# unknownue/puflow

Measured on AMD Instinct MI355X. Metric: patches/sec x4 2048->8192 (PU1K discrete, eval), higher is better.
Workload: dtype f32 (split-fp16 MFMA products, fp32 accumulate); 1 GPU; BASELINE configs[1]: PU1K discrete x4 inference, 32 x 2048-pt patches per GPU (fp32-parity mode); patches_per_gpu=32, total_batch=32, npoint=2048

## Files before the change

### include/puflow_hip.h

```cpp
#ifndef PUFLOW_HIP_H
#define PUFLOW_HIP_H

#ifdef __cplusplus
extern "C" {
#endif

#define PF_OK 0
#define PF_ERR_NULL (-1)
#define PF_ERR_SHAPE (-2)
#define PF_ERR_UNSUPPORTED (-3)
#define PF_ERR_LAUNCH (-4)
#define PF_ERR_WORKSPACE (-5)

int pf_version(void);
const char* pf_error_string(int code);

int pf_knn(const float* p1, const float* p2, int B, int N, int M, int K, int* idx_out, float* dist_out, void* stream);

int pf_nn1(const float* p1, const float* p2, int B, int N, int M, float* dist_out, int* idx_out, void* stream);

int pf_edgeconv(int cfg, const float* pq_or_xyz, const float* tab, const int* idx, const float* wfrag, float* out,
                int B, int N, void* stream);

int pf_edgeconv_tuned(int cfg, int variant, const float* pq_or_xyz, const float* tab, const int* idx,
                      const float* wfrag, float* out, int B, int N, void* stream);

int pf_edgeconv_pq(int unit, const float* pq_or_xyz, const int* idx, const float* wfrag, float* out, const float* w,
                   const long long* off, float* pq_next, int B, int N, int fuse, void* stream);

int pf_pq_gemm(int unit, const float* h, const float* w, const long long* off, float* pq_next, int T, void* stream);
int pf_cond(int unit, const float* h, const float* w, const long long* off, float* c, float* st, float* cp, int T,
            void* stream);
int pf_post(int unit, const float* h, const float* w, const long long* off, float* c, float* st, float* cp,
            float* pq_next, int T, void* stream);
int pf_test_act_pairn(const float* x, int n, float inv, float slope, unsigned* old_h, unsigned* old_l, unsigned* new_h,
                      unsigned* new_l, void* stream);
int pf_cond_all(const float* const* h, const float* w, const long long* off, float* const* c, float* st, float* cp, int T,
                void* stream);

int pf_flow_fwd(const float* xyz, const float* cp, const float* st, const float* w, float* z, float* ld_pt, int T,
                void* stream);

int pf_flow_inv(const float* u, const float* cp, const float* st, const float* w, float* x, int T, int R, void* stream);

int pf_logp(const float* z, const float* ld_pt, float ld_const, int B, int N, float* ldj, float* lpsum, float* logp,
            void* stream);

long long pf_flow_fwd_logp_ws_floats(int B, int N);
int pf_flow_fwd_logp(const float* xyz, const float* cp, const float* st, const float* w, float* z, float* ld_pt,
                     float ld_const, int B, int N, float* ldj, float* lpsum, float* logp, float* ws, void* stream);

int pf_interp(const float* xyz, const float* z, const int* idx16, const float* w, const long long* off, float* u_out,
              int B, int N, int R, void* stream);

int pf_interp_weights(const float* xyz, const int* idx16, const float* w, const long long* off, float* aw_out, int B, int N,
                      void* stream);
int pf_flow_inv_interp(const float* aw, const float* z, const int* idx16, const float* cp, const float* st, const float* w,
                       float* x, int B, int N, int R, void* stream);

int pf_chamfer_fwd(const float* x, const float* y, int B, int N, int M, float* dist1, int* idx1, float* dist2,
                   int* idx2, float* per_sample, float* mean_sum, void* stream);

int pf_chamfer_bwd(const float* x, const float* y, const int* idx1, const int* idx2, const float* g1, const float* g2,
                   float* gx, float* gy, int B, int N, int M, void* stream);
int pf_chamfer_bwd_det(const float* x, const float* y, const int* idx1, const int* idx2, const float* g1, const float* g2,
                       float* gx, float* gy, int B, int N, int M, void* stream);

int pf_emd_forward(const float* xyz1, const float* xyz2, float* dist, int* assignment, float* price,
                   int* assignment_inv, int* bid, float* bid_increments, float* max_increments, int* unass_idx,
                   int* max_idx, float eps, int iters, int B, int n, void* stream);

int pf_emd_forward_ex(const float* xyz1, const float* xyz2, float* dist, int* assignment, float* price,
                      int* assignment_inv, int* bid, float* bid_increments, float* max_increments, int* unass_idx,
                      int* max_idx, float eps, int iters, int B, int n, int groups, unsigned* status, void* stream);

int pf_emd_backward(const float* xyz1, const float* xyz2, float* gradxyz, const float* graddist, const int* idx, int B,
                    int n, void* stream);


long long pf_gemm_ws_floats(int M, int N, int K);
int pf_gemm(const float* A, long long sam, long long sak, const float* B, long long sbk, long long sbn, float* C,
// ... 405 lines not shown
```

### puflow_amd/csrc/flow.hip

```cpp
#include <hip/hip_runtime.h>
#include "pf_api_internal.h"
#include "pf_mfma.h"
#include "pf_wave.h"

#ifndef PF_FLOW_NW
#define PF_FLOW_NW 16
#endif
#ifndef PF_FLOW_NW_FWD
#define PF_FLOW_NW_FWD 16
#endif

namespace {

constexpr int FLOW_REC = 5360;
constexpr float LOG2PI_F = 1.8378770664093453f;

struct FlowArgs {
    const float* in;
    const float* cp;
    const float* st;
    const float* w;
    float* out;
    float* ld_pt;
    int T;
// ... 40 lines not shown
            v.z = fmaf(wb.x, h1[0], v.z); v.w = fmaf(wb.z, h1[0], v.w);
            if (TD == 2) {
                v.x = fmaf(wa.y, h1[1], v.x); v.y = fmaf(wa.w, h1[1], v.y);
                v.z = fmaf(wb.y, h1[1], v.z); v.w = fmaf(wb.w, h1[1], v.w);
            }
            hid[cb] = v;
        }
        hp[0][0] = pf_act_pairn(hid[0], hid[1], 0.01f);
        hp[0][1] = pf_act_pairn(hid[2], hid[3], 0.01f);
    }
    const PfW2Lds ws{reinterpret_cast<const u4*>(rec), lane};
    f4 h2[1][4];
#pragma unroll
    for (int ob = 0; ob < 4; ++ob) h2[0][ob] = pf_bias(rec + 5120, ob, q);
    pf_mmn<false, 4, 2, 2>(ws, 0, hp, h2);
    hp[0][0] = pf_act_pairn(h2[0][0], h2[0][1], i2, 0.01f);
    hp[0][1] = pf_act_pairn(h2[0][2], h2[0][3], i2, 0.01f);
    f4 acc[1][1];
    acc[0][0] = *reinterpret_cast<const f4*>(rec + 5184 + 4 * q);
    pf_mmn<false, 1, 2, 2>(ws, 8, hp, acc);
    o[0] = acc[0][0].x * i4; o[1] = acc[0][0].y * i4;
}

template <bool INV, int NW>
__global__ __launch_bounds__(NW * 64) void flow_kernel(FlowArgs a) {
    const int lane = threadIdx.x & 63, wave = threadIdx.x >> 6;
    const int col = lane & 15, q = lane >> 4;
    __shared__ f4 wl[6 * FLOW_REC / 4];
    pf_stage_lds(wl, reinterpret_cast<const f4*>(a.w), 6 * FLOW_REC / 4);
    __syncthreads();
    const float* wlf = reinterpret_cast<const float*>(wl);

    for (int tile = blockIdx.x; tile < a.ntiles; tile += gridDim.x) {
        const int g = (tile * NW + wave) * 16 + col;
        const bool ok = g < a.rows;
        const int row = ok ? g : a.rows - 1;
        const int pt = row / a.R;
        float v[3], ld = 0.f;
        if (INV && a.aw) {
            const int r = row - pt * a.R, bN = (pt / a.N) * a.N;
            const int4 j0 = *reinterpret_cast<const int4*>(a.idx + (size_t)pt * 16), j1 = *reinterpret_cast<const int4*>(a.idx + (size_t)pt * 16 + 4);
            const int jj[8] = {j0.x, j0.y, j0.z, j0.w, j1.x, j1.y, j1.z, j1.w};
            float sk[8][3];
#pragma unroll
            for (int k = 0; k < 8; ++k) {
                const float wk = a.aw[((size_t)pt * 8 + k) * 4 + r];
                const float* zz = a.z + (size_t)(bN + jj[k]) * 3;
// ... 10 lines not shown
        }
        FlowCond cn = flow_cond(a.cp, a.st, a.T, INV ? 5 : 0, pt, q);

        pf_static_for<0, 6>([&](auto uc) {
            constexpr int i = decltype(uc)::value;
            constexpr int u = INV ? 5 - i : i;
            constexpr int TD = (u % 2 == 0) ? 1 : 2;
            const float* rec = wlf + u * FLOW_REC;
            const float* fc = rec + 5328;
            const FlowCond c = cn;
            if constexpr (i < 5) cn = flow_cond(a.cp, a.st, a.T, INV ? u - 1 : u + 1, pt, q);
            __builtin_amdgcn_sched_barrier(0);
            const float s[3] = {c.s0.x, c.s0.y, c.s0.z}, t[3] = {c.s0.w, c.s1.x, c.s1.y};
            float h1[2], o[2];
            if constexpr (!INV) {
                const float x0 = v[0], x1 = v[1], x2 = v[2];
#pragma unroll
                for (int k = 0; k < 3; ++k)
                    v[k] = fmaf(fc[3 * k + 2], x2, fmaf(fc[3 * k + 1], x1, fmaf(fc[3 * k], x0, fc[9 + k])));
                h1[0] = v[0]; h1[1] = v[1];
                coupling_net<TD>(rec, lane, q, c, h1, o);
                if (TD == 1) { v[1] -= o[0]; v[2] -= o[1]; } else { v[2] -= o[0]; }
                const float y0 = v[2], y1 = v[1], y2 = v[0];
                v[0] = (y0 - t[0]) * expf(-s[0]);
                v[1] = (y1 - t[1]) * expf(-s[1]);
                v[2] = (y2 - t[2]) * expf(-s[2]);
                ld -= (s[0] + s[1]) + s[2];
            } else {
                const float y0 = fmaf(v[0], expf(s[0]), t[0]);
                const float y1 = fmaf(v[1], expf(s[1]), t[1]);
                const float y2 = fmaf(v[2], expf(s[2]), t[2]);
                v[0] = y2; v[1] = y1; v[2] = y0;
                h1[0] = v[0]; h1[1] = v[1];
                coupling_net<TD>(rec, lane, q, c, h1, o);
                if (TD == 1) { v[1] += o[0]; v[2] += o[1]; } else { v[2] += o[0]; }
                const float x0 = v[0], x1 = v[1], x2 = v[2];
#pragma unroll
                for (int k = 0; k < 3; ++k)
                    v[k] = fmaf(fc[12 + 3 * k + 2], x2, fmaf(fc[12 + 3 * k + 1], x1, fmaf(fc[12 + 3 * k], x0, fc[21 + k])));
            }
        });

        if (ok && q == 0) {
            a.out[(size_t)row * 3 + 0] = v[0];
            a.out[(size_t)row * 3 + 1] = v[1];
            a.out[(size_t)row * 3 + 2] = v[2];
            if (!INV) a.ld_pt[row] = ld;
        }
        if constexpr (!INV) {
            if (a.part) {
                float sl = ld;
                float sz = -0.5f * (v[0] * v[0] + LOG2PI_F) + -0.5f * (v[1] * v[1] + LOG2PI_F) + -0.5f * (v[2] * v[2] + LOG2PI_F);
                sl += __shfl_xor(sl, 1); sz += __shfl_xor(sz, 1);
                sl += __shfl_xor(sl, 2); sz += __shfl_xor(sz, 2);
// ... 23 lines not shown
            for (int i = lane; i < per; i += 64) {
                accl += PF_LD(a.part + b * per + i);
                accz += PF_LD(a.part + half + b * per + i);
            }
            accl = pf_xor_sum<32, 1>(accl); accz = pf_xor_sum<32, 1>(accz);
            if (lane == 0) {
                const float l = accl + a.ld_const * (float)a.N;
                a.ldj[b] = l;
                a.lps[b] = accz + l;
                if (b < NW * 64) sa[b] = accz + l;
            }
        }
        __syncthreads();
        float tot = 0.f;
        if (tid == 0)
            for (int b = 0; b < a.B; ++b) tot += b < NW * 64 ? sa[b] : a.lps[b];
        if (tid == 0) {
            *a.logp = -tot / (float)a.B;
            PF_ST(a.counter, 0u);
        }
    }
}

template <bool INV, int NW>
int launch_nw(FlowArgs a, hipStream_t s) {
    a.ntiles = (a.rows + NW * 16 - 1) / (NW * 16);
    const int grid = a.ntiles < 256 ? a.ntiles : 256;
    hipLaunchKernelGGL((flow_kernel<INV, NW>), dim3(grid), dim3(NW * 64), 0, s, a);
    return pf_last_launch_status();
}

template <bool INV>
int launch(FlowArgs a, hipStream_t s) {
    constexpr int NWMAX = INV ? PF_FLOW_NW : PF_FLOW_NW_FWD;
    const int wt = (a.rows + 15) / 16;
    if (wt >= 200 * NWMAX) return launch_nw<INV, NWMAX>(a, s);
    if (wt >= 200 * 8) return launch_nw<INV, 8>(a, s);
    return launch_nw<INV, 4>(a, s);
}

__global__ __launch_bounds__(256) void logp_batch_kernel(const float* __restrict__ z, const float* __restrict__ ld_pt,
                                                        float ld_const, int N, float* __restrict__ ldj,
                                                        float* __restrict__ lpsum) {
    __shared__ float sa[256], sb[256];
    const int b = blockIdx.x, tid = threadIdx.x;
    float accl = 0.f, accz = 0.f;
    for (int n = tid; n < N; n += 256) {
        accl += ld_pt[(size_t)b * N + n];
        const float* zz = z + ((size_t)b * N + n) * 3;
        accz += -0.5f * (zz[0] * zz[0] + LOG2PI_F) + -0.5f * (zz[1] * zz[1] + LOG2PI_F) + -0.5f * (zz[2] * zz[2] + LOG2PI_F);
    }
    sa[tid] = accl; sb[tid] = accz;
    __syncthreads();
    for (int s = 128; s > 0; s >>= 1) {
        if (tid < s) { sa[tid] += sa[tid + s]; sb[tid] += sb[tid + s]; }
        __syncthreads();
    }
    if (tid == 0) {
        const float l = sa[0] + ld_const * (float)N;
        ldj[b] = l;
        lpsum[b] = sb[0] + l;
    }
}

__global__ void logp_final_kernel(const float* __restrict__ lpsum, int B, float* __restrict__ logp) {
    if (threadIdx.x == 0 && blockIdx.x == 0) {
        float s = 0.f;
        for (int b = 0; b < B; ++b) s += lpsum[b];
        *logp = -s / (float)B;
    }
}

}

extern "C" int pf_flow_fwd(const float* xyz, const float* cp, const float* st, const float* w, float* z, float* ld_pt,
                           int T, void* stream) {
    if (!xyz || !cp || !st || !w || !z || !ld_pt) return PF_ERR_NULL;
    if (T <= 0) return PF_ERR_SHAPE;
    FlowArgs a{};
    a.in = xyz; a.cp = cp; a.st = st; a.w = w; a.out = z; a.ld_pt = ld_pt; a.T = T; a.R = 1; a.rows = T;
    return launch<false>(a, (hipStream_t)stream);
}

extern "C" long long pf_flow_fwd_logp_ws_floats(int B, int N) { return 2ll * (((long long)B * N + 15) / 16) + 4; }

extern "C" int pf_flow_fwd_logp(const float* xyz, const float* cp, const float* st, const float* w, float* z, float* ld_pt,
                                float ld_const, int B, int N, float* ldj, float* lpsum, float* logp, float* ws, void* stream) {
    if (!xyz || !cp || !st || !w || !z || !ld_pt || !ldj || !lpsum || !logp || !ws) return PF_ERR_NULL;
    if (B <= 0 || N <= 0 || (long long)B * N > (1ll << 30)) return PF_ERR_SHAPE;
    const int T = B * N;
    if (N % 16 != 0) {
        const int rc = pf_flow_fwd(xyz, cp, st, w, z, ld_pt, T, stream);
        return rc != PF_OK ? rc : pf_logp(z, ld_pt, ld_const, B, N, ldj, lpsum, logp, stream);
    }
    FlowArgs a{};
    a.in = xyz; a.cp = cp; a.st = st; a.w = w; a.out = z; a.ld_pt = ld_pt; a.T = T; a.R = 1; a.rows = T;
    a.part = ws; a.counter = reinterpret_cast<unsigned*>(ws + 2 * (T / 16));
    a.ldj = ldj; a.lps = lpsum; a.logp = logp; a.ld_const = ld_const; a.B = B; a.N = N;
    return launch<false>(a, (hipStream_t)stream);
}

extern "C" int pf_flow_inv(const float* u, const float* cp, const float* st, const float* w, float* x, int T, int R,
                           void* stream) {
    if (!u || !cp || !st || !w || !x) return PF_ERR_NULL;
    if (T <= 0 || R <= 0 || (long long)T * R > (1ll << 30)) return PF_ERR_SHAPE;
    FlowArgs a{};
    a.in = u; a.cp = cp; a.st = st; a.w = w; a.out = x; a.ld_pt = nullptr; a.T = T; a.R = R; a.rows = T * R;
    return launch<true>(a, (hipStream_t)stream);
}

extern "C" int pf_flow_inv_interp(const float* aw, const float* z, const int* idx16, const float* cp, const float* st, const float* w,
                                  float* x, int B, int N, int R, void* stream) {
    if (!aw || !z || !idx16 || !cp || !st || !w || !x) return PF_ERR_NULL;
    if (B <= 0 || N < 8 || (long long)B * N * R > (1ll << 30)) return PF_ERR_SHAPE;
    if (R < 1 || R > 4) return PF_ERR_UNSUPPORTED;
    FlowArgs a{};
    a.in = nullptr; a.cp = cp; a.st = st; a.w = w; a.out = x; a.ld_pt = nullptr; a.T = B * N; a.R = R; a.rows = B * N * R;
    a.aw = aw; a.z = z; a.idx = idx16; a.N = N;
    return launch<true>(a, (hipStream_t)stream);
}

extern "C" int pf_logp(const float* z, const float* ld_pt, float ld_const, int B, int N, float* ldj, float* lpsum,
                       float* logp, void* stream) {
    if (!z || !ld_pt || !ldj || !lpsum || !logp) return PF_ERR_NULL;
    if (B <= 0 || N <= 0) return PF_ERR_SHAPE;
    hipStream_t s = (hipStream_t)stream;
    hipLaunchKernelGGL(logp_batch_kernel, dim3(B), dim3(256), 0, s, z, ld_pt, ld_const, N, ldj, lpsum);
    hipLaunchKernelGGL(logp_final_kernel, dim3(1), dim3(64), 0, s, lpsum, B, logp);
    return pf_last_launch_status();
}
```

### puflow_amd/csrc/interp.hip

```cpp
#include <hip/hip_runtime.h>
#include "pf_api_internal.h"
#include "pf_mfma.h"
#include "pf_wave.h"

#ifndef PF_INTERP_P
#define PF_INTERP_P 1
#endif
#ifndef PF_INTERP_NW
#define PF_INTERP_NW 12
#endif

namespace {

struct InterpArgs {
    const float* xyz;
    const float* z;
    const int* idx;
    const float* w;
    long long off[15];
    float* u;
    float* aw;
    int T, N, ntiles, R;
    int per;
    int contiguous;
};

template <int P, int NW, bool BIG = false>
__global__ __launch_bounds__(NW * 64) void interp_kernel(InterpArgs a) {
    constexpr int R = 4;
    const int lane = threadIdx.x & 63, wave = threadIdx.x >> 6;
    const int col = lane & 15, q = lane >> 4;
    const int ps = col >> 3, k = col & 7;
    constexpr int L_DT = 0, L_ET = 2, L_WT = 6, L_D3 = 10, L_EC = 18, L_D6 = 34, L_W3 = 50, L_END = 66;
    __shared__ u4 wl[L_END * 128];
    {
        auto stage = [&](int f0, int nf, long long off) {
            const u4* src = reinterpret_cast<const u4*>(a.w + off);
            pf_stage_lds(wl + f0 * 128, src, nf * 128);
        };
        if (a.contiguous) stage(L_DT, L_END, a.off[0]);
        else {
            stage(L_DT, 2, a.off[0]); stage(L_ET, 4, a.off[5]); stage(L_WT, 4, a.off[8]); stage(L_D3, 8, a.off[1]);
            stage(L_EC, 16, a.off[6]); stage(L_D6, 16, a.off[3]); stage(L_W3, 16, a.off[9]);
        }
        __syncthreads();
    }
    const PfW1Lds wsDT{wl + L_DT * 128, lane}, wsET{wl + L_ET * 128, lane}, wsWT{wl + L_WT * 128, lane};
    const PfW2Lds wsD3{wl + L_D3 * 128, lane}, wsEC{wl + L_EC * 128, lane}, wsD6{wl + L_D6 * 128, lane}, wsW3{wl + L_W3 * 128, lane};
    const PfW2BufD<4> wsW0(a.w + a.off[7], lane);
    const PfW2BufD<2> wsW6(a.w + a.off[BIG ? 13 : 11], lane);

    const float* sc = a.w + a.off[4];
    const float iDT = sc[0], iD3 = sc[1], iW1 = sc[2], iEC = sc[3], iW3 = sc[4], iW6 = sc[5];

    const int wt_end = min((int)(blockIdx.x + 1) * a.per, a.ntiles);
    for (int wt = blockIdx.x * a.per + wave; wt < wt_end; wt += NW) {
        const int pt0 = wt * P * 2;
        int gi[P], gj[P];
        bool ok[P];
        h8 e[P];
#pragma unroll
        for (int p = 0; p < P; ++p) {
            const int g = pt0 + p * 2 + ps;
            ok[p] = g < a.T;
            gi[p] = ok[p] ? g : a.T - 1;
            gj[p] = (gi[p] / a.N) * a.N + a.idx[(size_t)gi[p] * 16 + k];
            float xi[3], xj[3];
#pragma unroll
            for (int c = 0; c < 3; ++c) {
                xi[c] = a.xyz[(size_t)gi[p] * 3 + c];
                xj[c] = a.xyz[(size_t)gj[p] * 3 + c];
            }
            const float v0 = xi[0] - xj[0], v1 = xi[1] - xj[1], v2 = xi[2] - xj[2];
            const float nrm = sqrtf(__fadd_rn(__fadd_rn(__fmul_rn(v0, v0), __fmul_rn(v1, v1)), __fmul_rn(v2, v2)));
            const f4 e0 = {xi[0], xi[1], xi[2], xj[0]}, e1 = {xj[1], xj[2], nrm, 1.f};
            e[p] = pf_edge_operand(e0, e1, q);
        }

        f4 w1[P][8];
// ... 193 lines not shown
```

### puflow_amd/csrc/pointwise.hip

```cpp
#include <hip/hip_runtime.h>
#include "pf_api_internal.h"
#include "pf_mfma.h"
#include "pf_pq.h"

namespace {

struct PqArgs {
    const float* h;
    const u4* w;
    const float* bias;
    const float* scales;
    float* pq;
    int T, ntiles, NT, nrounds;
    float inv;
};

template <int ODIM, int ROWS, int NW>
__global__ __launch_bounds__(NW * 64) void pq_gemm_kernel(PqArgs a) {
    constexpr int HB = ODIM / 16, CP = (HB + 1) / 2, OBT = ROWS / 16, RB = OBT / NW, NTMAX = 16;
    static_assert(OBT % NW == 0, "rows split evenly over the waves");
    const int lane = threadIdx.x & 63, wave = threadIdx.x >> 6;
    const int col = lane & 15, q = lane >> 4;
    __shared__ u4 bl[NTMAX * PQ_TILE_U4<CP>];
    h8 wh[RB][CP], wl[RB][CP];
// ... 25 lines not shown
        __syncthreads();
    }
}

template <int ODIM, int ROWS, int NW>
int launch_pq(PqArgs a, hipStream_t s) {
    a.ntiles = (a.T + 15) / 16;
    int nt = a.ntiles / 256;
    nt = nt < 1 ? 1 : (nt > 16 ? 16 : nt);
    a.NT = nt;
    a.nrounds = (a.ntiles + nt - 1) / nt;
    const int grid = a.nrounds < 256 ? a.nrounds : 256;
    hipLaunchKernelGGL((pq_gemm_kernel<ODIM, ROWS, NW>), dim3(grid), dim3(NW * 64), 0, s, a);
    return pf_last_launch_status();
}

struct CondArgs {
    const float* h;
    const float* w;
    long long off[13];
    float* c;
    float* st;
    float* cp;
    int T, ntiles;
    int contiguous;
};

__device__ __forceinline__ f4 pf_scale(f4 v, float k) { return v * k; }

template <int ODIM>
constexpr int cond_lds_bytes() { return ((ODIM / 32) * ((ODIM / 16 + 1) / 2) + 12 * ((ODIM / 32 + 1) / 2) + 20) * 2048; }

template <int ODIM, int CDIM, int NW>
__device__ __forceinline__ void cond_body(const CondArgs& a, u4* wl, int tile0, int tstride) {
    constexpr int HB = ODIM / 16, MB = ODIM / 32, CB = CDIM / 16;
    constexpr int HP = (HB + 1) / 2, MP = (MB + 1) / 2;
    constexpr int F_M1 = 0, F_H1 = F_M1 + MB * HP, F_S2 = F_H1 + 12 * MP, F_T2 = F_S2 + 8, F_ST4 = F_T2 + 8, F_END = F_ST4 + 4;
    const int lane = threadIdx.x & 63, wave = threadIdx.x >> 6;
    const int col = lane & 15, q = lane >> 4;
    static_assert(F_END * 2048 == cond_lds_bytes<ODIM>(), "LDS size formula");
    {
        auto stage = [&](int f0, int nf, long long off) {
            const u4* src = reinterpret_cast<const u4*>(a.w + off);
            pf_stage_lds(wl + f0 * 128, src, nf * 128);
        };
        if (a.contiguous) stage(F_M1, F_END, a.off[0]);
// ... 30 lines not shown
        }
        PfPairN mp[1][MP];
        {
            f4 m[1][MB + (MB & 1)];
#pragma unroll
            for (int o = 0; o < MB; ++o) m[0][o] = pf_bias(b1, o, q);
            pf_mmn<false, MB, HP, HP>(wsM1, 0, hp, m);
#pragma unroll
            for (int c = 0; c < MP; ++c) {
                if (2 * c + 1 < MB) mp[0][c] = pf_relu_pairn(m[0][2 * c], m[0][2 * c + 1], iM1);
                else mp[0][c] = pf_join_halfn(pf_relu_halfn(m[0][2 * c], iM1), PfHalfN{});
            }
        }
        if (a.c) {
            f4 c[1][CB];
#pragma unroll
            for (int o = 0; o < CB; ++o) c[0][o] = pf_splat(0.f);
            pf_mmn<false, CB, MP, MP>(wsM2, 0, mp, c);
            if (ok)
#pragma unroll
                for (int o = 0; o < CB; ++o)
                    *reinterpret_cast<f4*>(a.c + (size_t)pt * CDIM + o * 16 + 4 * q) = pf_scale(c[0][o], iM2);
        }
        if (!a.st) continue;
        {
            f4 acc[1][4];
#pragma unroll
            for (int o = 0; o < 4; ++o) acc[0][o] = pf_splat(0.f);
            pf_mmn<false, 4, MP, MP>(wsH1, 8 * MP, mp, acc);
            if (ok)
#pragma unroll
                for (int o = 0; o < 4; ++o)
                    *reinterpret_cast<f4*>(a.cp + (size_t)pt * 64 + o * 16 + 4 * q) = pf_scale(acc[0][o], iH1);
        }
        PfPairN h2p[1][4];
        pf_static_for<0, 2>([&](auto nc) {
            constexpr int net = decltype(nc)::value;
            f4 h1[1][4];
#pragma unroll
            for (int o = 0; o < 4; ++o) h1[0][o] = pf_splat(0.f);
            pf_mmn<false, 4, MP, MP>(wsH1, (4 * net) * MP, mp, h1);
            PfPairN h1p[1][2];
            h1p[0][0] = pf_act_pairn(h1[0][0], h1[0][1], iH1, 0.01f);
            h1p[0][1] = pf_act_pairn(h1[0][2], h1[0][3], iH1, 0.01f);
            f4 h2[1][4];
#pragma unroll
            for (int o = 0; o < 4; ++o) h2[0][o] = pf_bias(net == 0 ? bS2 : bT2, o, q);
            if constexpr (net == 0) pf_mmn<false, 4, 2, 2>(wsS2, 0, h1p, h2); else pf_mmn<false, 4, 2, 2>(wsT2, 0, h1p, h2);
            const float i2 = net == 0 ? iS2 : iT2;
            h2p[0][2 * net + 0] = pf_act_pairn(h2[0][0], h2[0][1], i2, 0.01f);
            h2p[0][2 * net + 1] = pf_act_pairn(h2[0][2], h2[0][3], i2, 0.01f);
        });
        {
            f4 acc[1][1];
            acc[0][0] = pf_bias(bST4, 0, q);
            pf_mmn<false, 1, 4, 4>(wsST4, 0, h2p, acc);
            if (ok && q < 2) *reinterpret_cast<f4*>(a.st + (size_t)pt * 8 + 4 * q) = pf_scale(acc[0][0], iST4);
        }
    }
}

#ifndef PF_COND_NW
#define PF_COND_NW 12
#endif
constexpr int COND_NW = PF_COND_NW;

template <int ODIM, int CDIM>
__global__ __launch_bounds__(COND_NW * 64) void cond_kernel(CondArgs a) {
    extern __shared__ u4 cond_lds[];
    cond_body<ODIM, CDIM, COND_NW>(a, cond_lds, blockIdx.x, gridDim.x);
}

struct CondAllArgs { CondArgs u[6]; int first[7]; };

__global__ __launch_bounds__(COND_NW * 64) void cond_all_kernel(CondAllArgs g) {
    extern __shared__ u4 cond_lds[];
    const int b = blockIdx.x;
    int unit = 0;
#pragma unroll
    for (int i = 1; i < 6; ++i) unit += b >= g.first[i] ? 1 : 0;
// ... 65 lines not shown
        case 32: return launch_pq<32, 288, 9>(a, s);
        case 64: return launch_pq<64, 288, 9>(a, s);
        case 128: return launch_pq<128, 288, 9>(a, s);
        default: return PF_ERR_UNSUPPORTED;
    }
}

extern "C" int pf_cond(int unit, const float* h, const float* w, const long long* off, float* c, float* st, float* cp,
                       int T, void* stream) {
    if (!h || !w || !off || !st || !cp) return PF_ERR_NULL;
    if (T <= 0) return PF_ERR_SHAPE;
    CondArgs a{};
    a.h = h; a.w = w; a.c = c; a.st = st; a.cp = cp; a.T = T;
    for (int i = 0; i < 13; ++i) a.off[i] = off[i];
    hipStream_t s = (hipStream_t)stream;
    switch (unit) {
        case 0: return launch_cond<32, 32>(a, s);
        case 1: return launch_cond<64, 64>(a, s);
        case 2: case 3: case 4: case 5: return launch_cond<128, 128>(a, s);
        default: return PF_ERR_UNSUPPORTED;
    }
}

extern "C" int pf_cond_all(const float* const* h, const float* w, const long long* off, float* const* c, float* st, float* cp,
                           int T, void* stream) {
    if (!h || !w || !off || (!st != !cp) || (!st && !c)) return PF_ERR_NULL;
    if (T <= 0) return PF_ERR_SHAPE;
    CondAllArgs g{};
    const int ntiles = (T + 15) / 16;
    const int wgt = (ntiles + COND_NW - 1) / COND_NW;
    static const int share_big[6] = {32, 32, 48, 48, 48, 48}, share_small[6] = {24, 32, 50, 50, 50, 50};
    const int* share = wgt <= 50 ? share_small : share_big;
    g.first[0] = 0;
    for (int u = 0; u < 6; ++u) {
        if (!h[u]) return PF_ERR_NULL;
        CondArgs& a = g.u[u];
        a.h = h[u]; a.w = w; a.c = c ? c[u] : nullptr; a.st = st ? st + (size_t)u * T * 8 : nullptr; a.cp = cp ? cp + (size_t)u * T * 64 : nullptr; a.T = T;
        a.ntiles = ntiles;
        for (int i = 0; i < 13; ++i) a.off[i] = off[u * 13 + i];
        a.contiguous = cond_contiguous(a.off, u == 0 ? 32 : (u == 1 ? 64 : 128));
        const int n = wgt < share[u] ? wgt : share[u];
        g.first[u + 1] = g.first[u] + n;
    }
    constexpr int lds = cond_lds_bytes<128>();
    allow_lds(cond_all_kernel, lds);
    hipLaunchKernelGGL(cond_all_kernel, dim3(g.first[6]), dim3(COND_NW * 64), lds, (hipStream_t)stream, g);
    return pf_last_launch_status();
}

extern "C" int pf_post(int unit, const float* h, const float* w, const long long* off, float* c, float* st, float* cp,
                       float* pq_next, int T, void* stream) {
    if (unit < 5) {
        if (!pq_next) return PF_ERR_NULL;
        const int rc = pf_pq_gemm(unit, h, w, off, pq_next, T, stream);
        if (rc != PF_OK) return rc;
    }
    return pf_cond(unit, h, w, off, c, st, cp, T, stream);
}

namespace {
__global__ void act_pairn_test_kernel(const float* __restrict__ x, int n8, float inv, float slope, u4* __restrict__ old_h,
                                      u4* __restrict__ old_l, u4* __restrict__ new_h, u4* __restrict__ new_l) {
    const int i = blockIdx.x * blockDim.x + threadIdx.x;
    if (i >= n8) return;
    const f4 b0 = *reinterpret_cast<const f4*>(x + (size_t)i * 8), b1 = *reinterpret_cast<const f4*>(x + (size_t)i * 8 + 4);
    const PfPairN o = pf_pairn(pf_lrelu(pf_scale(b0, inv), slope), pf_lrelu(pf_scale(b1, inv), slope));
    const PfPairN n = inv == 1.f ? pf_act_pairn(b0, b1, slope) : pf_act_pairn(b0, b1, inv, slope);
    old_h[i] = __builtin_bit_cast(u4, o.h); old_l[i] = __builtin_bit_cast(u4, o.l);
    new_h[i] = __builtin_bit_cast(u4, n.h); new_l[i] = __builtin_bit_cast(u4, n.l);
}
// ... 13 lines not shown
```

### puflow_amd/interpflow.py

```python
from __future__ import annotations

import os
from typing import List, Optional, Tuple

import numpy as np
import torch
import torch.nn as nn
from torch import Tensor

from . import _lib
from .packing import COND_CHANNELS, FEAT_CHANNELS, GROWTH, NUM_BLOCKS, fold_state_dict, pack_plan

_EC_CFG = [0, 1, 2, 2, 2, 2]
_CHECK_FINITE = os.environ.get("PF_CHECK_FINITE", "0") == "1"


def _conv_bn(cin: int, cout: int, slope: float) -> nn.Sequential:
    return nn.Sequential(nn.Conv2d(cin, cout, kernel_size=1), nn.BatchNorm2d(cout), nn.LeakyReLU(slope))


class _EdgeConvParams(nn.Module):

    def __init__(self, cin: int, odim: int, growth: int):
        super().__init__()
        nconv = odim // growth
        self.convs = nn.ModuleList([_conv_bn(3 * cin + growth * t, growth, 0.05) for t in range(nconv)])
# ... 50 lines not shown
        self.coupling1.bias_net = _CondNet(tdim + cdim, hdim, idim - tdim)
        self.coupling2 = _Holder()
        self.coupling2.bias_net = _CondNet(cdim, hdim, idim)
        self.coupling2.scale_net = _CondNet(cdim, hdim, idim)


class _InterpParams(nn.Module):

    def __init__(self):
        super().__init__()
        self.knn_context = _Holder()
        self.knn_context.distance_encoder = _Holder()
        self.knn_context.distance_encoder.mlp = nn.Sequential(
            *_conv_bn(10, 64, 0.01), *_conv_bn(64, 64, 0.01), nn.Conv2d(64, 128, kernel_size=1))
        self.knn_context.feat_conv = _EdgeConvParams(3, 128, 16)
        self.weight_unit = _Holder()
        self.weight_unit.mlp = nn.Sequential(
            *_conv_bn(256, 128, 0.01), *_conv_bn(128, 64, 0.01), nn.Conv2d(64, 32, kernel_size=1))


class CondList(list):
    cp: Tensor
    st: Tensor


def _host_state_dict(sd):
    out, groups = {}, {}
    for k, v in sd.items():
        v = v.detach()
        if v.is_cuda:
            groups.setdefault(v.dtype, []).append((k, v))
        else:
            out[k] = v
    for dt, items in groups.items():
        flat = torch.cat([v.reshape(-1) for _, v in items]).cpu()
        pos = 0
        for k, v in items:
            out[k] = flat[pos:pos + v.numel()].reshape(v.shape)
            pos += v.numel()
    return {k: out[k] for k in sd}


class _Engine:
    def __init__(self, sd, device: torch.device, ec_mode: Optional[str] = None):
        sd = _host_state_dict(sd)
        self.lib = _lib.load()
# ... 51 lines not shown
        for u in range(NUM_BLOCKS):
            h = torch.empty((T, FEAT_CHANNELS[u + 1]), dtype=torch.float32, device=dev)
            src = xyz.data_ptr() if u == 0 else (pq if u % 2 else pq2).data_ptr()
            nxt = pq2 if u % 2 else pq

            def ec(u=u, src=src, h=h):
                self._edgeconv(u, src, idx16, h, B, N, s)

            def ec_pq(u=u, src=src, h=h, nxt=nxt):
                w = self.ec1n_w[u] if u < 2 else self.ec4_w[u]
                _lib.check(self.lib.pf_edgeconv_pq(u, src, idx16.data_ptr(), self._p(w), h.data_ptr(), self.base, self.post[u],
                                                   nxt.data_ptr(), B, N, self.fuse_pq, s), f"pf_edgeconv_pq[{u}]")

            def pq_gemm(u=u, h=h, nxt=nxt):
                _lib.check(self.lib.pf_pq_gemm(u, h.data_ptr(), self.base, self.post[u], nxt.data_ptr(), T, s), f"pf_pq_gemm[{u}]")

            if u + 1 == NUM_BLOCKS:
                yield h, [(f"edgeconv{u}", ec)]
            elif fused:
                yield h, [(f"edgeconv{u}+pq", ec_pq)]
            else:
                yield h, [(f"edgeconv{u}", ec), (f"pq{u}", pq_gemm)]

    def features(self, xyz: Tensor, idx16: Tensor, want_cs: bool, cs_only: bool = False):
        B, N, _ = xyz.shape
        T, dev, s = B * N, xyz.device, self._stream()
        cp = torch.empty((NUM_BLOCKS, T, 64), dtype=torch.float32, device=dev) if not (cs_only and want_cs) else None
        st = torch.empty((NUM_BLOCKS, T, 8), dtype=torch.float32, device=dev) if not (cs_only and want_cs) else None
        hs: List[Tensor] = []
        for h, calls in self._unit_chain(xyz, idx16):
            for _, call in calls:
                call()
            hs.append(h)
        cs: List[Optional[Tensor]] = [torch.empty((B, N, COND_CHANNELS[u]), dtype=torch.float32, device=dev) if want_cs else None
                                      for u in range(NUM_BLOCKS)]
        self._cond_all(hs, cs if want_cs else None, st, cp, T, s)
        return (cs if want_cs else None), cp, st

    def _cond_all(self, hs, cs, st: Optional[Tensor], cp: Optional[Tensor], T: int, s) -> None:
        import ctypes
        PtrArr = ctypes.c_void_p * NUM_BLOCKS
        h_arr = PtrArr(*[h.data_ptr() for h in hs])
        c_arr = PtrArr(*[c.data_ptr() for c in cs]) if cs is not None else None
        _lib.check(self.lib.pf_cond_all(h_arr, self.base, self.post_all, c_arr, st.data_ptr() if st is not None else None,
                                        cp.data_ptr() if cp is not None else None, T, s), "pf_cond_all")

    def logp_ws(self, B: int, N: int, dev) -> Tensor:
        return torch.zeros((int(self.lib.pf_flow_fwd_logp_ws_floats(B, N)),), dtype=torch.float32, device=dev)

    def flow_f(self, xyz: Tensor, cp: Tensor, st: Tensor, ws: Optional[Tensor] = None):
        B, N, _ = xyz.shape
        T, dev, s = B * N, xyz.device, self._stream()
        z = torch.empty((B, N, 3), dtype=torch.float32, device=dev)
        ld_pt = torch.empty((T,), dtype=torch.float32, device=dev)
        ldj = torch.empty((B,), dtype=torch.float32, device=dev)
        lps = torch.empty((B,), dtype=torch.float32, device=dev)
        logp = torch.empty((), dtype=torch.float32, device=dev)
        if ws is None:
            key = (B, N, s)
            ws = self._logp_ws.get(key)
            if ws is None:
                ws = self._logp_ws[key] = self.logp_ws(B, N, dev)
        _lib.check(self.lib.pf_flow_fwd_logp(xyz.data_ptr(), cp.data_ptr(), st.data_ptr(), self._p(self.flow), z.data_ptr(),
                                             ld_pt.data_ptr(), self.ld_const, B, N, ldj.data_ptr(), lps.data_ptr(), logp.data_ptr(),
                                             ws.data_ptr(), s), "pf_flow_fwd_logp")
        return z, ldj, logp

    def interp(self, xyz: Tensor, z: Tensor, idx16: Tensor, R: int) -> Tensor:
        B, N, _ = xyz.shape
        u = torch.empty((B, N * R, 3), dtype=torch.float32, device=xyz.device)
        _lib.check(self.lib.pf_interp(xyz.data_ptr(), z.data_ptr(), idx16.data_ptr(), self.base, self.interp_off,
                                      u.data_ptr(), B, N, R, self._stream()), "pf_interp")
        return u

    def interp_weights(self, xyz: Tensor, idx16: Tensor) -> Tensor:
        B, N, _ = xyz.shape
        aw = torch.empty((B * N, 8, 4), dtype=torch.float32, device=xyz.device)
        _lib.check(self.lib.pf_interp_weights(xyz.data_ptr(), idx16.data_ptr(), self.base, self.interp_off, aw.data_ptr(), B, N,
                                              self._stream()), "pf_interp_weights")
        return aw

    def flow_g_interp(self, aw: Tensor, z: Tensor, idx16: Tensor, cp: Tensor, st: Tensor, R: int) -> Tensor:
        B, N, _ = z.shape
        x = torch.empty((B, N * R, 3), dtype=torch.float32, device=z.device)
        _lib.check(self.lib.pf_flow_inv_interp(aw.data_ptr(), z.data_ptr(), idx16.data_ptr(), cp.data_ptr(), st.data_ptr(),
                                               self._p(self.flow), x.data_ptr(), B, N, R, self._stream()), "pf_flow_inv_interp")
        return x

    def side_stream(self) -> "torch.cuda.Stream":
        if self._side is None:
            self._side = torch.cuda.Stream(device=self.device)
        return self._side

    def split_interp_for(self, T: int, R: int) -> bool:
        return R <= 4 and self.split_interp == 1

    def flow_g(self, u: Tensor, cp: Tensor, st: Tensor, R: int) -> Tensor:
        B, NR, _ = u.shape
        T = B * NR // R
        x = torch.empty_like(u)
        _lib.check(self.lib.pf_flow_inv(u.data_ptr(), cp.data_ptr(), st.data_ptr(), self._p(self.flow), x.data_ptr(),
                                        T, R, self._stream()), "pf_flow_inv")
        return x


    def profile_stages(self, xyz: Tensor, iters: int = 5, R: int = 4) -> dict:
        B, N, _ = xyz.shape
        T, dev, s = B * N, xyz.device, self._stream()
        acc: dict = {}

        def timed(name, fn):
            a, b = torch.cuda.Event(enable_timing=True), torch.cuda.Event(enable_timing=True)
            a.record()
            r = fn()
            b.record()
            acc.setdefault(name, []).append((a, b))
            return r

        for _ in range(iters + 1):
            idx16 = timed("knn", lambda: self.knn(xyz))
            cp = torch.empty((NUM_BLOCKS, T, 64), dtype=torch.float32, device=dev)
            st = torch.empty((NUM_BLOCKS, T, 8), dtype=torch.float32, device=dev)
            hs = []
            for h, calls in self._unit_chain(xyz, idx16, split_two_launch=True):
                for name, call in calls:
# ... 108 lines not shown
        u = torch.flatten(self._prep(z).transpose(2, 3), 1, 2).contiguous()
        return self._engine(upratio).flow_g(u, cs.cp, cs.st, upratio)

    def forward(self, xyz: Tensor, upratio: int = 4) -> Tuple[Tensor, Tensor]:
        if self.training:
            from .train_ops import forward_train
            if not xyz.is_cuda:
                raise _lib.PuflowHipError("input must be a GPU tensor (no CPU fallback)")
            self._train_forwards = getattr(self, "_train_forwards", 0) + 1
            return forward_train(self, xyz, upratio)
        with torch.no_grad():
            return self._forward_eval(xyz, upratio)

    def _forward_eval(self, xyz: Tensor, upratio: int, ws: Optional[Tensor] = None) -> Tuple[Tensor, Tensor]:
        self._check_mode()
        xyz = self._prep(xyz)
        e = self._engine(upratio)
        idx16 = e.knn(xyz)
        if e.split_interp_for(xyz.shape[0] * xyz.shape[1], upratio):
            main, side = torch.cuda.current_stream(), e.side_stream()
            side.wait_stream(main)
            with torch.cuda.stream(side):
                aw = e.interp_weights(xyz, idx16)
            _, cp, st = e.features(xyz, idx16, want_cs=False)
            z, _, logp = e.flow_f(xyz, cp, st, ws)
            main.wait_stream(side)
            aw.record_stream(main)
            x = e.flow_g_interp(aw, z, idx16, cp, st, upratio)
        else:
            _, cp, st = e.features(xyz, idx16, want_cs=False)
            z, _, logp = e.flow_f(xyz, cp, st, ws)
            u = e.interp(xyz, z, idx16, upratio)
            x = e.flow_g(u, cp, st, upratio)
        if _CHECK_FINITE and not bool(torch.isfinite(x).all() & torch.isfinite(logp)):
            raise _lib.PuflowHipError("non-finite output: an activation left the fp16 range of the split-fp16 kernels "
                                      "(or the input holds NaN/inf); check the input normalisation (patch.py:168-178)")
        return x, logp

    @torch.no_grad()
    def forward_stages(self, xyz: Tensor, upratio: int = 4) -> dict:
        self._check_mode()
        xyz = self._prep(xyz)
        e = self._engine(upratio)
        idx16 = e.knn(xyz)
        cs, cp, st = e.features(xyz, idx16, want_cs=True)
        z, ldj, logp = e.flow_f(xyz, cp, st)
        u = e.interp(xyz, z, idx16, upratio)
        x = e.flow_g(u, cp, st, upratio)
        B, N, _ = xyz.shape
        fz = u.view(B, N, upratio, 3).transpose(2, 3)
        return dict(idx16=idx16, cs=cs, cp=cp, st=st, z=z, ldj=ldj, logp=logp, fz=fz, x=x)

    def sample(self, sparse: Tensor, upratio: int = 4) -> Tensor:
# ... 40 lines not shown
```

Before: 28520 patches/s.

## Precompute flow scale exponentials and log-det in cond kernel; dynamic interp tile scheduling

The conditioning kernel now also writes per-point records holding exp(s) or exp(-s), the shift terms and the summed log-determinant, in separate forward and inverse layouts. The forward and inverse flow kernels read these records instead of calling expf per coupling step, and the inverse runs R times per point, so the same exponentials were being recomputed. The interp kernel also switches from a static per-wave tile stride to an LDS atomic counter for dynamic tile assignment. This adds two extra T×8 record buffers per block to write and read, and the atomic adds some contention.

```diff
diff --git a/include/puflow_hip.h b/include/puflow_hip.h
--- a/include/puflow_hip.h
+++ b/include/puflow_hip.h
@@ -37,6 +37,8 @@
                       unsigned* new_l, void* stream);
 int pf_cond_all(const float* const* h, const float* w, const long long* off, float* const* c, float* st, float* cp, int T,
                 void* stream);
+int pf_cond_all_rec(const float* const* h, const float* w, const long long* off, float* const* c, float* st, float* cp,
+                    float* rec_f, float* rec_g, int T, void* stream);
 
 int pf_flow_fwd(const float* xyz, const float* cp, const float* st, const float* w, float* z, float* ld_pt, int T,
                 void* stream);
@@ -57,6 +59,13 @@
                       void* stream);
 int pf_flow_inv_interp(const float* aw, const float* z, const int* idx16, const float* cp, const float* st, const float* w,
                        float* x, int B, int N, int R, void* stream);
+
+int pf_flow_fwd_logp_rec(const float* xyz, const float* cp, const float* rec_f, const float* w, float* z, float* ld_pt,
+                         float ld_const, int B, int N, float* ldj, float* lpsum, float* logp, float* ws, void* stream);
+int pf_flow_inv_rec(const float* u, const float* cp, const float* rec_g, const float* w, float* x, int T, int R, void* stream);
+int pf_flow_inv_interp_rec(const float* aw, const float* z, const int* idx16, const float* cp, const float* rec_g,
+                           const float* w, float* x, int B, int N, int R, void* stream);
+int pf_test_flow_expf(const float* x, int n, float* y, void* stream);
 
 int pf_chamfer_fwd(const float* x, const float* y, int B, int N, int M, float* dist1, int* idx1, float* dist2,
                    int* idx2, float* per_sample, float* mean_sum, void* stream);
diff --git a/puflow_amd/csrc/flow.hip b/puflow_amd/csrc/flow.hip
--- a/puflow_amd/csrc/flow.hip
+++ b/puflow_amd/csrc/flow.hip
@@ -86,7 +86,7 @@
     o[0] = acc[0][0].x * i4; o[1] = acc[0][0].y * i4;
 }
 
-template <bool INV, int NW>
+template <bool INV, bool REC, int NW>
 __global__ __launch_bounds__(NW * 64) void flow_kernel(FlowArgs a) {
     const int lane = threadIdx.x & 63, wave = threadIdx.x >> 6;
     const int col = lane & 15, q = lane >> 4;
@@ -143,14 +143,21 @@
                 coupling_net<TD>(rec, lane, q, c, h1, o);
                 if (TD == 1) { v[1] -= o[0]; v[2] -= o[1]; } else { v[2] -= o[0]; }
                 const float y0 = v[2], y1 = v[1], y2 = v[0];
-                v[0] = (y0 - t[0]) * expf(-s[0]);
-                v[1] = (y1 - t[1]) * expf(-s[1]);
-                v[2] = (y2 - t[2]) * expf(-s[2]);
-                ld -= (s[0] + s[1]) + s[2];
+                if constexpr (REC) {
+                    v[0] = (y0 - t[0]) * s[0];
+                    v[1] = (y1 - t[1]) * s[1];
+                    v[2] = (y2 - t[2]) * s[2];
+                    ld += c.s1.z;
+                } else {
+                    v[0] = (y0 - t[0]) * expf(-s[0]);
+                    v[1] = (y1 - t[1]) * expf(-s[1]);
+                    v[2] = (y2 - t[2]) * expf(-s[2]);
+                    ld -= (s[0] + s[1]) + s[2];
+                }
             } else {
-                const float y0 = fmaf(v[0], expf(s[0]), t[0]);
-                const float y1 = fmaf(v[1], expf(s[1]), t[1]);
-                const float y2 = fmaf(v[2], expf(s[2]), t[2]);
+                const float y0 = fmaf(v[0], REC ? s[0] : expf(s[0]), t[0]);
+                const float y1 = fmaf(v[1], REC ? s[1] : expf(s[1]), t[1]);
+                const float y2 = fmaf(v[2], REC ? s[2] : expf(s[2]), t[2]);
                 v[0] = y2; v[1] = y1; v[2] = y0;
                 h1[0] = v[0]; h1[1] = v[1];
                 coupling_net<TD>(rec, lane, q, c, h1, o);
@@ -220,21 +227,26 @@
     }
 }
 
-template <bool INV, int NW>
+template <bool INV, bool REC, int NW>
 int launch_nw(FlowArgs a, hipStream_t s) {
     a.ntiles = (a.rows + NW * 16 - 1) / (NW * 16);
     const int grid = a.ntiles < 256 ? a.ntiles : 256;
-    hipLaunchKernelGGL((flow_kernel<INV, NW>), dim3(grid), dim3(NW * 64), 0, s, a);
+    hipLaunchKernelGGL((flow_kernel<INV, REC, NW>), dim3(grid), dim3(NW * 64), 0, s, a);
     return pf_last_launch_status();
 }
 
-template <bool INV>
-int launch(FlowArgs a, hipStream_t s) {
+template <bool INV, bool REC>
+int launch_rec(FlowArgs a, hipStream_t s) {
     constexpr int NWMAX = INV ? PF_FLOW_NW : PF_FLOW_NW_FWD;
     const int wt = (a.rows + 15) / 16;
-    if (wt >= 200 * NWMAX) return launch_nw<INV, NWMAX>(a, s);
-    if (wt >= 200 * 8) return launch_nw<INV, 8>(a, s);
-    return launch_nw<INV, 4>(a, s);
+    if (wt >= 200 * NWMAX) return launch_nw<INV, REC, NWMAX>(a, s);
+    if (wt >= 200 * 8) return launch_nw<INV, REC, 8>(a, s);
+    return launch_nw<INV, REC, 4>(a, s);
+}
+
+template <bool INV>
+int launch(FlowArgs a, bool rec, hipStream_t s) {
+    return rec ? launch_rec<INV, true>(a, s) : launch_rec<INV, false>(a, s);
 }
 
 __global__ __launch_bounds__(256) void logp_batch_kernel(const float* __restrict__ z, const float* __restrict__ ld_pt,
@@ -271,51 +283,100 @@
 
 }
 
-extern "C" int pf_flow_fwd(const float* xyz, const float* cp, const float* st, const float* w, float* z, float* ld_pt,
-                           int T, void* stream) {
+static int flow_fwd(const float* xyz, const float* cp, const float* st, bool rec, const float* w, float* z, float* ld_pt,
+                    int T, void* stream) {
     if (!xyz || !cp || !st || !w || !z || !ld_pt) return PF_ERR_NULL;
     if (T <= 0) return PF_ERR_SHAPE;
     FlowArgs a{};
     a.in = xyz; a.cp = cp; a.st = st; a.w = w; a.out = z; a.ld_pt = ld_pt; a.T = T; a.R = 1; a.rows = T;
-    return launch<false>(a, (hipStream_t)stream);
+    return launch<false>(a, rec, (hipStream_t)stream);
+}
+
+extern "C" int pf_flow_fwd(const float* xyz, const float* cp, const float* st, const float* w, float* z, float* ld_pt,
+                           int T, void* stream) {
+    return flow_fwd(xyz, cp, st, false, w, z, ld_pt, T, stream);
 }
 
 extern "C" long long pf_flow_fwd_logp_ws_floats(int B, int N) { return 2ll * (((long long)B * N + 15) / 16) + 4; }
 
-extern "C" int pf_flow_fwd_logp(const float* xyz, const float* cp, const float* st, const float* w, float* z, float* ld_pt,
-                                float ld_const, int B, int N, float* ldj, float* lpsum, float* logp, float* ws, void* stream) {
+static int flow_fwd_logp(const float* xyz, const float* cp, const float* st, bool rec, const float* w, float* z, float* ld_pt,
+                         float ld_const, int B, int N, float* ldj, float* lpsum, float* logp, float* ws, void* stream) {
     if (!xyz || !cp || !st || !w || !z || !ld_pt || !ldj || !lpsum || !logp || !ws) return PF_ERR_NULL;
     if (B <= 0 || N <= 0 || (long long)B * N > (1ll << 30)) return PF_ERR_SHAPE;
     const int T = B * N;
     if (N % 16 != 0) {
-        const int rc = pf_flow_fwd(xyz, cp, st, w, z, ld_pt, T, stream);
+        const int rc = flow_fwd(xyz, cp, st, rec, w, z, ld_pt, T, stream);
         return rc != PF_OK ? rc : pf_logp(z, ld_pt, ld_const, B, N, ldj, lpsum, logp, stream);
     }
     FlowArgs a{};
     a.in = xyz; a.cp = cp; a.st = st; a.w = w; a.out = z; a.ld_pt = ld_pt; a.T = T; a.R = 1; a.rows = T;
     a.part = ws; a.counter = reinterpret_cast<unsigned*>(ws + 2 * (T / 16));
     a.ldj = ldj; a.lps = lpsum; a.logp = logp; a.ld_const = ld_const; a.B = B; a.N = N;
-    return launch<false>(a, (hipStream_t)stream);
-}
-
-extern "C" int pf_flow_inv(const float* u, const float* cp, const float* st, const float* w, float* x, int T, int R,
-                           void* stream) {
+    return launch<false>(a, rec, (hipStream_t)stream);
+}
+
+extern "C" int pf_flow_fwd_logp(const float* xyz, const float* cp, const float* st, const float* w, float* z, float* ld_pt,
+                                float ld_const, int B, int N, float* ldj, float* lpsum, float* logp, float* ws, void* stream) {
+    return flow_fwd_logp(xyz, cp, st, false, w, z, ld_pt, ld_const, B, N, ldj, lpsum, logp, ws, stream);
+}
+
+extern "C" int pf_flow_fwd_logp_rec(const float* xyz, const float* cp, const float* rec_f, const float* w, float* z, float* ld_pt,
+                                    float ld_const, int B, int N, float* ldj, float* lpsum, float* logp, float* ws, void* stream) {
+    return flow_fwd_logp(xyz, cp, rec_f, true, w, z, ld_pt, ld_const, B, N, ldj, lpsum, logp, ws, stream);
+}
+
+static int flow_inv(const float* u, const float* cp, const float* st, bool rec, const float* w, float* x, int T, int R,
+                    void* stream) {
     if (!u || !cp || !st || !w || !x) return PF_ERR_NULL;
     if (T <= 0 || R <= 0 || (long long)T * R > (1ll << 30)) return PF_ERR_SHAPE;
     FlowArgs a{};
     a.in = u; a.cp = cp; a.st = st; a.w = w; a.out = x; a.ld_pt = nullptr; a.T = T; a.R = R; a.rows = T * R;
-    return launch<true>(a, (hipStream_t)stream);
-}
-
-extern "C" int pf_flow_inv_interp(const float* aw, const float* z, const int* idx16, const float* cp, const float* st, const float* w,
-                                  float* x, int B, int N, int R, void* stream) {
+    return launch<true>(a, rec, (hipStream_t)stream);
+}
+
+extern "C" int pf_flow_inv(const float* u, const float* cp, const float* st, const float* w, float* x, int T, int R,
+                           void* stream) {
+    return flow_inv(u, cp, st, false, w, x, T, R, stream);
+}
+
+extern "C" int pf_flow_inv_rec(const float* u, const float* cp, const float* rec_g, const float* w, float* x, int T, int R,
+                               void* stream) {
+    return flow_inv(u, cp, rec_g, true, w, x, T, R, stream);
+}
+
+static int flow_inv_interp(const float* aw, const float* z, const int* idx16, const float* cp, const float* st, bool rec,
+                           const float* w, float* x, int B, int N, int R, void* stream) {
     if (!aw || !z || !idx16 || !cp || !st || !w || !x) return PF_ERR_NULL;
     if (B <= 0 || N < 8 || (long long)B * N * R > (1ll << 30)) return PF_ERR_SHAPE;
     if (R < 1 || R > 4) return PF_ERR_UNSUPPORTED;
     FlowArgs a{};
     a.in = nullptr; a.cp = cp; a.st = st; a.w = w; a.out = x; a.ld_pt = nullptr; a.T = B * N; a.R = R; a.rows = B * N * R;
     a.aw = aw; a.z = z; a.idx = idx16; a.N = N;
-    return launch<true>(a, (hipStream_t)stream);
+    return launch<true>(a, rec, (hipStream_t)stream);
+}
+
+extern "C" int pf_flow_inv_interp(const float* aw, const float* z, const int* idx16, const float* cp, const float* st, const float* w,
+                                  float* x, int B, int N, int R, void* stream) {
+    return flow_inv_interp(aw, z, idx16, cp, st, false, w, x, B, N, R, stream);
+}
+
+extern "C" int pf_flow_inv_interp_rec(const float* aw, const float* z, const int* idx16, const float* cp, const float* rec_g,
+                                      const float* w, float* x, int B, int N, int R, void* stream) {
+    return flow_inv_interp(aw, z, idx16, cp, rec_g, true, w, x, B, N, R, stream);
+}
+
+namespace {
+__global__ void flow_expf_test_kernel(const float* __restrict__ x, int n, float* __restrict__ y) {
+    const int i = blockIdx.x * blockDim.x + threadIdx.x;
+    if (i < n) y[i] = expf(x[i]);
+}
+}
+
+extern "C" int pf_test_flow_expf(const float* x, int n, float* y, void* stream) {
+    if (!x || !y) return PF_ERR_NULL;
+    if (n <= 0) return PF_ERR_SHAPE;
+    hipLaunchKernelGGL(flow_expf_test_kernel, dim3((n + 255) / 256), dim3(256), 0, (hipStream_t)stream, x, n, y);
+    return pf_last_launch_status();
 }
 
 extern "C" int pf_logp(const float* z, const float* ld_pt, float ld_const, int B, int N, float* ldj, float* lpsum,
diff --git a/puflow_amd/csrc/interp.hip b/puflow_amd/csrc/interp.hip
--- a/puflow_amd/csrc/interp.hip
+++ b/puflow_amd/csrc/interp.hip
@@ -33,6 +33,7 @@
     const int ps = col >> 3, k = col & 7;
     constexpr int L_DT = 0, L_ET = 2, L_WT = 6, L_D3 = 10, L_EC = 18, L_D6 = 34, L_W3 = 50, L_END = 66;
     __shared__ u4 wl[L_END * 128];
+    __shared__ int next_wt;
     {
         auto stage = [&](int f0, int nf, long long off) {
             const u4* src = reinterpret_cast<const u4*>(a.w + off);
@@ -43,6 +44,7 @@
             stage(L_DT, 2, a.off[0]); stage(L_ET, 4, a.off[5]); stage(L_WT, 4, a.off[8]); stage(L_D3, 8, a.off[1]);
             stage(L_EC, 16, a.off[6]); stage(L_D6, 16, a.off[3]); stage(L_W3, 16, a.off[9]);
         }
+        if (threadIdx.x == 0) next_wt = NW;
         __syncthreads();
     }
     const PfW1Lds wsDT{wl + L_DT * 128, lane}, wsET{wl + L_ET * 128, lane}, wsWT{wl + L_WT * 128, lane};
@@ -54,7 +56,12 @@
     const float iDT = sc[0], iD3 = sc[1], iW1 = sc[2], iEC = sc[3], iW3 = sc[4], iW6 = sc[5];
 
     const int wt_end = min((int)(blockIdx.x + 1) * a.per, a.ntiles);
-    for (int wt = blockIdx.x * a.per + wave; wt < wt_end; wt += NW) {
+    auto next_tile = [&]() {
+        int i = 0;
+        if (lane == 0) i = atomicAdd(&next_wt, 1);
+        return (int)blockIdx.x * a.per + __builtin_amdgcn_readfirstlane(i);
+    };
+    for (int wt = blockIdx.x * a.per + wave; wt < wt_end; wt = next_tile()) {
         const int pt0 = wt * P * 2;
         int gi[P], gj[P];
         bool ok[P];
diff --git a/puflow_amd/csrc/pointwise.hip b/puflow_amd/csrc/pointwise.hip
--- a/puflow_amd/csrc/pointwise.hip
+++ b/puflow_amd/csrc/pointwise.hip
@@ -71,6 +71,8 @@
     float* c;
     float* st;
     float* cp;
+    float* rec_f;
+    float* rec_g;
     int T, ntiles;
     int contiguous;
 };
@@ -147,7 +149,7 @@
                 for (int o = 0; o < CB; ++o)
                     *reinterpret_cast<f4*>(a.c + (size_t)pt * CDIM + o * 16 + 4 * q) = pf_scale(c[0][o], iM2);
         }
-        if (!a.st) continue;
+        if (!a.cp) continue;
         {
             f4 acc[1][4];
 #pragma unroll
@@ -180,7 +182,20 @@
             f4 acc[1][1];
             acc[0][0] = pf_bias(bST4, 0, q);
             pf_mmn<false, 1, 4, 4>(wsST4, 0, h2p, acc);
-            if (ok && q < 2) *reinterpret_cast<f4*>(a.st + (size_t)pt * 8 + 4 * q) = pf_scale(acc[0][0], iST4);
+            const f4 stv = pf_scale(acc[0][0], iST4);
+            if (a.st && ok && q < 2) *reinterpret_cast<f4*>(a.st + (size_t)pt * 8 + 4 * q) = stv;
+            if (a.rec_f) {
+                const float s0 = __shfl(stv.x, col), s1 = __shfl(stv.y, col), s2 = __shfl(stv.z, col), t0 = __shfl(stv.w, col);
+                const float e0 = expf(q == 1 ? -s0 : s0), e1 = expf(q == 1 ? -s1 : s1), e2 = expf(q == 1 ? -s2 : s2);
+                const f4 lo = {e0, e1, e2, t0};
+                if (ok && q == 0) *reinterpret_cast<f4*>(a.rec_g + (size_t)pt * 8) = lo;
+                if (ok && q == 1) {
+                    const f4 gh = {stv.x, stv.y, 0.f, 0.f}, fh = {stv.x, stv.y, -((s0 + s1) + s2), 0.f};
+                    *reinterpret_cast<f4*>(a.rec_g + (size_t)pt * 8 + 4) = gh;
+                    *reinterpret_cast<f4*>(a.rec_f + (size_t)pt * 8) = lo;
+                    *reinterpret_cast<f4*>(a.rec_f + (size_t)pt * 8 + 4) = fh;
+                }
+            }
         }
     }
 }
@@ -292,9 +307,8 @@
     }
 }
 
-extern "C" int pf_cond_all(const float* const* h, const float* w, const long long* off, float* const* c, float* st, float* cp,
-                           int T, void* stream) {
-    if (!h || !w || !off || (!st != !cp) || (!st && !c)) return PF_ERR_NULL;
+static int cond_all_launch(const float* const* h, const float* w, const long long* off, float* const* c, float* st, float* cp,
+                           float* rec_f, float* rec_g, int T, void* stream) {
     if (T <= 0) return PF_ERR_SHAPE;
     CondAllArgs g{};
     const int ntiles = (T + 15) / 16;
@@ -306,6 +320,7 @@
         if (!h[u]) return PF_ERR_NULL;
         CondArgs& a = g.u[u];
         a.h = h[u]; a.w = w; a.c = c ? c[u] : nullptr; a.st = st ? st + (size_t)u * T * 8 : nullptr; a.cp = cp ? cp + (size_t)u * T * 64 : nullptr; a.T = T;
+        a.rec_f = rec_f ? rec_f + (size_t)u * T * 8 : nullptr; a.rec_g = rec_g ? rec_g + (size_t)u * T * 8 : nullptr;
         a.ntiles = ntiles;
         for (int i = 0; i < 13; ++i) a.off[i] = off[u * 13 + i];
         a.contiguous = cond_contiguous(a.off, u == 0 ? 32 : (u == 1 ? 64 : 128));
@@ -316,6 +331,18 @@
     allow_lds(cond_all_kernel, lds);
     hipLaunchKernelGGL(cond_all_kernel, dim3(g.first[6]), dim3(COND_NW * 64), lds, (hipStream_t)stream, g);
     return pf_last_launch_status();
+}
+
+extern "C" int pf_cond_all(const float* const* h, const float* w, const long long* off, float* const* c, float* st, float* cp,
+                           int T, void* stream) {
+    if (!h || !w || !off || (!st != !cp) || (!st && !c)) return PF_ERR_NULL;
+    return cond_all_launch(h, w, off, c, st, cp, nullptr, nullptr, T, stream);
+}
+
+extern "C" int pf_cond_all_rec(const float* const* h, const float* w, const long long* off, float* const* c, float* st, float* cp,
+                               float* rec_f, float* rec_g, int T, void* stream) {
+    if (!h || !w || !off || !cp || !rec_f || !rec_g) return PF_ERR_NULL;
+    return cond_all_launch(h, w, off, c, st, cp, rec_f, rec_g, T, stream);
 }
 
 extern "C" int pf_post(int unit, const float* h, const float* w, const long long* off, float* c, float* st, float* cp,
diff --git a/puflow_amd/interpflow.py b/puflow_amd/interpflow.py
--- a/puflow_amd/interpflow.py
+++ b/puflow_amd/interpflow.py
@@ -1,7 +1,7 @@
 from __future__ import annotations
 
 import os
-from typing import List, Optional, Tuple
+from typing import List, NamedTuple, Optional, Tuple
 
 import numpy as np
 import torch
@@ -98,6 +98,11 @@
 class CondList(list):
     cp: Tensor
     st: Tensor
+
+
+class CondRecords(NamedTuple):
+    f: Tensor
+    g: Tensor
 
 
 def _host_state_dict(sd):
@@ -195,11 +200,13 @@
             else:
                 yield h, [(f"edgeconv{u}", ec), (f"pq{u}", pq_gemm)]
 
-    def features(self, xyz: Tensor, idx16: Tensor, want_cs: bool, cs_only: bool = False):
+    def features(self, xyz: Tensor, idx16: Tensor, want_cs: bool, cs_only: bool = False, records: bool = False):
         B, N, _ = xyz.shape
         T, dev, s = B * N, xyz.device, self._stream()
         cp = torch.empty((NUM_BLOCKS, T, 64), dtype=torch.float32, device=dev) if not (cs_only and want_cs) else None
-        st = torch.empty((NUM_BLOCKS, T, 8), dtype=torch.float32, device=dev) if not (cs_only and want_cs) else None
+        st = torch.empty((NUM_BLOCKS, T, 8), dtype=torch.float32, device=dev) if not (cs_only and want_cs or records) else None
+        rec = CondRecords(torch.empty((NUM_BLOCKS, T, 8), dtype=torch.float32, device=dev),
+                          torch.empty((NUM_BLOCKS, T, 8), dtype=torch.float32, device=dev)) if records else None
         hs: List[Tensor] = []
         for h, calls in self._unit_chain(xyz, idx16):
             for _, call in calls:
@@ -207,16 +214,20 @@
             hs.append(h)
         cs: List[Optional[Tensor]] = [torch.empty((B, N, COND_CHANNELS[u]), dtype=torch.float32, device=dev) if want_cs else None
                                       for u in range(NUM_BLOCKS)]
-        self._cond_all(hs, cs if want_cs else None, st, cp, T, s)
-        return (cs if want_cs else None), cp, st
-
-    def _cond_all(self, hs, cs, st: Optional[Tensor], cp: Optional[Tensor], T: int, s) -> None:
+        self._cond_all(hs, cs if want_cs else None, st, cp, T, s, rec)
+        return (cs if want_cs else None), cp, (rec if records else st)
+
+    def _cond_all(self, hs, cs, st: Optional[Tensor], cp: Optional[Tensor], T: int, s, rec: Optional[CondRecords] = None) -> None:
         import ctypes
         PtrArr = ctypes.c_void_p * NUM_BLOCKS
         h_arr = PtrArr(*[h.data_ptr() for h in hs])
         c_arr = PtrArr(*[c.data_ptr() for c in cs]) if cs is not None else None
-        _lib.check(self.lib.pf_cond_all(h_arr, self.base, self.post_all, c_arr, st.data_ptr() if st is not None else None,
-                                        cp.data_ptr() if cp is not None else None, T, s), "pf_cond_all")
+        st_p, cp_p = (st.data_ptr() if st is not None else None), (cp.data_ptr() if cp is not None else None)
+        if rec is not None:
+            _lib.check(self.lib.pf_cond_all_rec(h_arr, self.base, self.post_all, c_arr, st_p, cp_p, rec.f.data_ptr(),
+                                                rec.g.data_ptr(), T, s), "pf_cond_all_rec")
+        else:
+            _lib.check(self.lib.pf_cond_all(h_arr, self.base, self.post_all, c_arr, st_p, cp_p, T, s), "pf_cond_all")
 
     def logp_ws(self, B: int, N: int, dev) -> Tensor:
         return torch.zeros((int(self.lib.pf_flow_fwd_logp_ws_floats(B, N)),), dtype=torch.float32, device=dev)
@@ -234,9 +245,10 @@
             ws = self._logp_ws.get(key)
             if ws is None:
                 ws = self._logp_ws[key] = self.logp_ws(B, N, dev)
-        _lib.check(self.lib.pf_flow_fwd_logp(xyz.data_ptr(), cp.data_ptr(), st.data_ptr(), self._p(self.flow), z.data_ptr(),
-                                             ld_pt.data_ptr(), self.ld_const, B, N, ldj.data_ptr(), lps.data_ptr(), logp.data_ptr(),
-                                             ws.data_ptr(), s), "pf_flow_fwd_logp")
+        fn, cond = (self.lib.pf_flow_fwd_logp_rec, st.f) if isinstance(st, CondRecords) else (self.lib.pf_flow_fwd_logp, st)
+        _lib.check(fn(xyz.data_ptr(), cp.data_ptr(), cond.data_ptr(), self._p(self.flow), z.data_ptr(),
+                      ld_pt.data_ptr(), self.ld_const, B, N, ldj.data_ptr(), lps.data_ptr(), logp.data_ptr(),
+                      ws.data_ptr(), s), "pf_flow_fwd_logp")
         return z, ldj, logp
 
     def interp(self, xyz: Tensor, z: Tensor, idx16: Tensor, R: int) -> Tensor:
@@ -256,8 +268,9 @@
     def flow_g_interp(self, aw: Tensor, z: Tensor, idx16: Tensor, cp: Tensor, st: Tensor, R: int) -> Tensor:
         B, N, _ = z.shape
         x = torch.empty((B, N * R, 3), dtype=torch.float32, device=z.device)
-        _lib.check(self.lib.pf_flow_inv_interp(aw.data_ptr(), z.data_ptr(), idx16.data_ptr(), cp.data_ptr(), st.data_ptr(),
-                                               self._p(self.flow), x.data_ptr(), B, N, R, self._stream()), "pf_flow_inv_interp")
+        fn, cond = (self.lib.pf_flow_inv_interp_rec, st.g) if isinstance(st, CondRecords) else (self.lib.pf_flow_inv_interp, st)
+        _lib.check(fn(aw.data_ptr(), z.data_ptr(), idx16.data_ptr(), cp.data_ptr(), cond.data_ptr(),
+                      self._p(self.flow), x.data_ptr(), B, N, R, self._stream()), "pf_flow_inv_interp")
         return x
 
     def side_stream(self) -> "torch.cuda.Stream":
@@ -272,8 +285,9 @@
         B, NR, _ = u.shape
         T = B * NR // R
         x = torch.empty_like(u)
-        _lib.check(self.lib.pf_flow_inv(u.data_ptr(), cp.data_ptr(), st.data_ptr(), self._p(self.flow), x.data_ptr(),
-                                        T, R, self._stream()), "pf_flow_inv")
+        fn, cond = (self.lib.pf_flow_inv_rec, st.g) if isinstance(st, CondRecords) else (self.lib.pf_flow_inv, st)
+        _lib.check(fn(u.data_ptr(), cp.data_ptr(), cond.data_ptr(), self._p(self.flow), x.data_ptr(),
+                      T, R, self._stream()), "pf_flow_inv")
         return x
 
 
@@ -428,13 +442,13 @@
             side.wait_stream(main)
             with torch.cuda.stream(side):
                 aw = e.interp_weights(xyz, idx16)
-            _, cp, st = e.features(xyz, idx16, want_cs=False)
+            _, cp, st = e.features(xyz, idx16, want_cs=False, records=True)
             z, _, logp = e.flow_f(xyz, cp, st, ws)
             main.wait_stream(side)
             aw.record_stream(main)
             x = e.flow_g_interp(aw, z, idx16, cp, st, upratio)
         else:
-            _, cp, st = e.features(xyz, idx16, want_cs=False)
+            _, cp, st = e.features(xyz, idx16, want_cs=False, records=True)
             z, _, logp = e.flow_f(xyz, cp, st, ws)
             u = e.interp(xyz, z, idx16, upratio)
             x = e.flow_g(u, cp, st, upratio)
```

New measurement: 28650 patches/s, median of 6. No clear change (+0.4%).
